# nv-tlabs/DiffusionTexturePainting

Hardware: AMD Instinct MI355X
Metric: 512x512 inpaint stamps/sec @20 DDIM steps (higher is better)
Workload: dtype f16

## Files before the change

### diffusiontexturepainting_amd/csrc/common.h

```cpp
#pragma once
#include <hip/hip_runtime.h>
#include <stdint.h>

#include "../../include/dtp.h"

typedef _Float16 f16;
typedef f16 f16x2 __attribute__((ext_vector_type(2)));
typedef f16 f16x4 __attribute__((ext_vector_type(4)));
typedef f16 f16x8 __attribute__((ext_vector_type(8)));
typedef float f32x4 __attribute__((ext_vector_type(4)));
typedef float f32x16 __attribute__((ext_vector_type(16)));

static __device__ __forceinline__ uint32_t lds_addr(const void* p) {
  return (uint32_t)(uintptr_t)(const __attribute__((address_space(3))) void*)p;
}
static __device__ __forceinline__ f16x8 lds_read16(uint32_t addr) {
  f16x8 v;
  asm volatile("ds_read_b128 %0, %1" : "=v"(v) : "v"(addr));
  return v;
}
template <int N, int NF>
static __device__ __forceinline__ void wait_lds_frags(f16x8 (&f)[NF]) {
  static_assert(NF == 2 || NF == 3 || NF == 4 || NF == 5 || NF == 6 || NF == 7 || NF == 8, "fragment count");
  if constexpr (NF == 2) asm volatile("s_waitcnt lgkmcnt(%2)" : "+v"(f[0]), "+v"(f[1]) : "n"(N));
  else if constexpr (NF == 3) asm volatile("s_waitcnt lgkmcnt(%3)" : "+v"(f[0]), "+v"(f[1]), "+v"(f[2]) : "n"(N));
  else if constexpr (NF == 4) asm volatile("s_waitcnt lgkmcnt(%4)" : "+v"(f[0]), "+v"(f[1]), "+v"(f[2]), "+v"(f[3]) : "n"(N));
  else if constexpr (NF == 5)
    asm volatile("s_waitcnt lgkmcnt(%5)" : "+v"(f[0]), "+v"(f[1]), "+v"(f[2]), "+v"(f[3]), "+v"(f[4]) : "n"(N));
  else if constexpr (NF == 6)
    asm volatile("s_waitcnt lgkmcnt(%6)" : "+v"(f[0]), "+v"(f[1]), "+v"(f[2]), "+v"(f[3]), "+v"(f[4]), "+v"(f[5]) : "n"(N));
  else if constexpr (NF == 7)
    asm volatile("s_waitcnt lgkmcnt(%7)"
                 : "+v"(f[0]), "+v"(f[1]), "+v"(f[2]), "+v"(f[3]), "+v"(f[4]), "+v"(f[5]), "+v"(f[6])
                 : "n"(N));
  else
    asm volatile("s_waitcnt lgkmcnt(%8)"
                 : "+v"(f[0]), "+v"(f[1]), "+v"(f[2]), "+v"(f[3]), "+v"(f[4]), "+v"(f[5]), "+v"(f[6]), "+v"(f[7])
                 : "n"(N));
}



#ifndef DTP_IEEE_DIV
static __device__ __forceinline__ float fast_rcp(float x) { return __builtin_amdgcn_rcpf(x); }
#else
static __device__ __forceinline__ float fast_rcp(float x) { return 1.0f / x; }
#endif
static __device__ __forceinline__ float silu_f(float x) { return x * fast_rcp(1.0f + __expf(-x)); }
static __device__ __forceinline__ float quick_gelu_f(float x) { return x * fast_rcp(1.0f + __expf(-1.702f * x)); }

#ifndef DTP_GELU_POLY
static __device__ __forceinline__ float gelu_erf(float x) {
  const float z = fabsf(x) * 0.70710678118654752f;
  const float t = fast_rcp(fmaf(0.3275911f, z, 1.0f));
  float pl = fmaf(1.061405429f, t, -1.453152027f);
  pl = fmaf(pl, t, 1.421413741f);
  pl = fmaf(pl, t, -0.284496736f);
  pl = fmaf(pl, t, 0.254829592f);
  const float e = 1.0f - pl * t * __expf(-z * z);
  return 0.5f * x * (1.0f + copysignf(e, x));
}
#else
static __device__ __forceinline__ float gelu_erf(float x) {
  const float z = fminf(fabsf(x) * 0.70710678118654752f, 3.0f);
  const float u = z * z;
  float p = fmaf(4.074155537e-08f, u, -1.944803169e-06f);
  p = fmaf(p, u, 4.106023957e-05f);
  p = fmaf(p, u, -5.110346811e-04f);
  p = fmaf(p, u, 4.235417930e-03f);
  p = fmaf(p, u, -2.510283806e-02f);
  p = fmaf(p, u, 1.110793054e-01f);
  p = fmaf(p, u, -3.753148582e-01f);
  p = fmaf(p, u, 1.128268424e+00f);
  const float h = 0.5f * x;
  return fmaf(fabsf(h), p * z, h);
}
#endif

typedef float f32x2 __attribute__((ext_vector_type(2)));
template <class T>
static __device__ __forceinline__ void sum_pairs_strided_t(const float* __restrict__ p, size_t stride, int n, T& s1, T& s2) {
  s1 = 0; s2 = 0;
  int q = 0;
  for (; q + 8 <= n; q += 8) {
    f32x2 t[8];
#pragma unroll
    for (int e = 0; e < 8; ++e) t[e] = *(const f32x2*)(p + (size_t)(q + e) * stride);
#pragma unroll
    for (int e = 0; e < 8; ++e) { s1 += (T)t[e][0]; s2 += (T)t[e][1]; }
  }
  if (q < n) {
    f32x2 t[8];
#pragma unroll
    for (int e = 0; e < 8; ++e) t[e] = *(const f32x2*)(p + (size_t)(q + (q + e < n ? e : 0)) * stride);
#pragma unroll
    for (int e = 0; e < 8; ++e)
      if (q + e < n) { s1 += (T)t[e][0]; s2 += (T)t[e][1]; }
  }
}
static __device__ __forceinline__ void sum_pairs_strided(const float* __restrict__ p, size_t stride, int n, float& s1, float& s2) {
  sum_pairs_strided_t(p, stride, n, s1, s2);
}
static __device__ __forceinline__ void sum_pairs_strided_d(const float* __restrict__ p, size_t stride, int n, double& s1, double& s2) {
  sum_pairs_strided_t(p, stride, n, s1, s2);
}
static __device__ __forceinline__ f32x4 col4(const float* __restrict__ v, int n, int N) {
  if (n + 4 <= N) return *(const f32x4*)(v + n);
  f32x4 r = {0.f, 0.f, 0.f, 0.f};
#pragma unroll
  for (int e = 0; e < 4; ++e)
    if (n + e < N) r[e] = v[n + e];
  return r;
}
static __device__ __forceinline__ double shfl_xor_d(double v, int o) {
  int lo = __double2loint(v), hi = __double2hiint(v);
  lo = __shfl_xor(lo, o); hi = __shfl_xor(hi, o);
  return __hiloint2double(hi, lo);
}
template <int CTRL>
static __device__ __forceinline__ float dpp_get_f(float v) {
  return __builtin_bit_cast(float, __builtin_amdgcn_update_dpp(0, __builtin_bit_cast(int, v), CTRL, 0xf, 0xf, false));
}
static __device__ __forceinline__ void swap16_f(float x, float& a, float& b) {
  a = x; b = x;
  asm volatile("s_nop 1\n\tv_permlane16_swap_b32 %0, %1" : "+v"(a), "+v"(b));
}
static __device__ __forceinline__ void swap32_f(float x, float& a, float& b) {
  a = x; b = x;
  asm volatile("s_nop 1\n\tv_permlane32_swap_b32 %0, %1" : "+v"(a), "+v"(b));
}
template <int W>
static __device__ __forceinline__ float group_allsum(float v) {
  static_assert(W == 2 || W == 4 || W == 8 || W == 16 || W == 32 || W == 64, "group width");
  v += dpp_get_f<0xb1>(v);
  if constexpr (W >= 4) v += dpp_get_f<0x4e>(v);
  if constexpr (W >= 8) v += dpp_get_f<0x141>(v);
  if constexpr (W >= 16) v += dpp_get_f<0x140>(v);
  if constexpr (W >= 32) { float a, b; swap16_f(v, a, b); v = a + b; }
  if constexpr (W >= 64) { float a, b; swap32_f(v, a, b); v = a + b; }
  return v;
}
template <int W>
static __device__ __forceinline__ float group_allmax(float v) {
  static_assert(W == 2 || W == 4 || W == 8 || W == 16, "group width");
  v = fmaxf(v, dpp_get_f<0xb1>(v));
  if constexpr (W >= 4) v = fmaxf(v, dpp_get_f<0x4e>(v));
  if constexpr (W >= 8) v = fmaxf(v, dpp_get_f<0x141>(v));
  if constexpr (W >= 16) v = fmaxf(v, dpp_get_f<0x140>(v));
  return v;
}
static __device__ __forceinline__ float xhalf_sum(float v) { float a, b; swap32_f(v, a, b); return a + b; }
static __device__ __forceinline__ float xhalf_max(float v) { float a, b; swap32_f(v, a, b); return fmaxf(a, b); }

template <int CTRL>
static __device__ __forceinline__ double dpp_add8_d(double v) {
  const int lo = __builtin_amdgcn_update_dpp(0, __double2loint(v), CTRL, 0xf, 0xf, false);
  const int hi = __builtin_amdgcn_update_dpp(0, __double2hiint(v), CTRL, 0xf, 0xf, false);
  return v + __hiloint2double(hi, lo);
}
static __device__ __forceinline__ double sum8_d(double v) {
  v = dpp_add8_d<0xb1>(v);
  v = dpp_add8_d<0x4e>(v);
  v = dpp_add8_d<0x141>(v);
  return v;
}
static __device__ __forceinline__ void gn_mean_rstd(double s, double q, float inv_count, float eps, float& mean, float& rstd) {
  const float nf = rintf(1.0f / inv_count);
  const double n = (double)nf;
  double inv = (double)(1.0f / nf);
  inv = inv * (2.0 - n * inv);
  const double m = s * inv;
  const double var = q * inv - m * m;
  mean = (float)m;
  rstd = rsqrtf(fmaxf((float)var, 0.f) + eps);
}

#define DTP_WAVE 64

#define HIP_CHECK(x)                                                                        \
  do {                                                                                      \
    hipError_t e_ = (x);                                                                    \
    if (e_ != hipSuccess) {                                                                 \
      dtp_set_error("%s:%d %s -> %s", __FILE__, __LINE__, #x, hipGetErrorString(e_));       \
      return DTP_ERR_HIP;                                                                   \
    }                                                                                       \
  } while (0)


void dtp_set_error(const char* fmt, ...);

enum {
  GF_BIAS = 1,
  GF_BIAS_M = 2,
  GF_RESID = 4,
  GF_GEGLU = 8,
  GF_CONV3 = 16,
  GF_UPS2 = 32,
  GF_GELU = 64,
  GF_QUICKGELU = 128,
  GF_OUT_F32 = 256,
  GF_SILU = 512,
  GF_LNFOLD = 1024,
  GF_ROWSTATS = 2048,
  GF_SOFTMAX16 = 4096,
  GF_MFAST = 1 << 20,
  GF_NOREDUCE = 1 << 21,
  GF_XCDSPLIT = 1 << 23,
  GF_GNSTATS = 1 << 24,
  GF_RAGGED = 1 << 25,
  GF_GNAPPLY = 1 << 22,
};

struct GemmParams {
  const f16* A;
  const f16* W;
  const f16* Wcb;
  const f16* Wfr;
  void* C;
  float* part;
  const float* bias;
  const f16* R;
  const f16* zero;
  const float* lns;
  float ln_eps;
  const float* st_in;
  int st_parts;
  float* st_out;
  int M, N, K;
  int lda, ldw, ldc, ldr;
  int nkb;
  int splits;
  int kb_per_split;
  int col_ranges;
  int Hi, Wi, Ho, Wo, Cin, stride, pad;
  const f16* A2;
  int lda2, Cin2;
  int flags;
  int batch;
  long long a_bs, w_bs, c_bs, r_bs;
  int bias_bs, lns_bs, st_rows;
  int sm_valid;
  const float *gn_part, *gn_gamma, *gn_beta;
  int gn_nchunk, gn_cpg, gn_silu;
  float gn_eps;
  const unsigned char* W8;
  int ldw8;
  float a_scale, w_scale;
  const float* a_scale_host;
  int amax_slot1;
  const unsigned char* A8;
  int lda8;
  const unsigned char* A2_8;
  int lda2_8;
  unsigned char* C8;
  int ldc8;
  float c_scale;
  float a2_scale;
};

struct Quant8Job {
  const f16* x; int ld, K;
  unsigned char* y; int ldy;
  float scale;
  int ln;
};
struct Quant8Params {
  int M, njobs;
  Quant8Job job[2];
  const float* st_in; int st_parts, st_rows;
  float eps;
};
bool dtp_quant8_supported(const Quant8Params& q);
int dtp_launch_quant8(const Quant8Params& q, hipStream_t s);
bool dtp_gemm_f8f8_supported(const GemmParams& p);
int dtp_gemm_f8f8_pick(const GemmParams& p, int num_cu);
int dtp_launch_gemm_f8f8(const GemmParams& p, int tile, hipStream_t s);
void dtp_gemm_f8f8_init();

static inline bool dtp_xcd_split_ok(int tiles, int splits) {
  if (splits < 2 || (splits & (splits - 1)) || splits > 32) return false;
  return splits >= 8 || (tiles % (8 / splits)) == 0;
}
static __device__ __forceinline__ void dtp_xcd_split(int id, int tiles, int splits, int& tile, int& z) {
  const int xcd = id & 7, idx = id >> 3;
  if (splits >= 8) { const int r = splits >> 3; z = xcd + 8 * (idx % r); tile = idx / r; }
  else { const int g = 8 / splits; z = xcd % splits; tile = idx * g + xcd / splits; }
}

int dtp_launch_gemm(const GemmParams& p, int tile, hipStream_t s);
void dtp_gemm_init();
int dtp_launch_tile(const GemmParams& p, int tile, hipStream_t s);
int dtp_launch_splitk_reduce(const GemmParams& p, hipStream_t s);
size_t dtp_gemm_workspace_bytes(const GemmParams& p);
void dtp_gemm_pick(GemmParams& p, int* tile, int num_cu);

struct GnParams {
  const f16* x; int ldx; f16* y; int ldy; const float *gamma, *beta; int B, HW, C, groups; float eps; int silu;
};
struct GnReduceSrc {
  const float* part; int splits; long long slab; int ldp; const float* bias; const f16* R; int ldr;
};
int dtp_launch_groupnorm(const GnParams& p, float* stats_ws, hipStream_t s);
size_t dtp_groupnorm_ws_bytes(int B, int HW, int C, int groups);
int dtp_groupnorm_stat_chunks(int HW);
int dtp_launch_groupnorm_apply(const GnParams& p, const float* partial, int nchunk, hipStream_t s);
int dtp_launch_groupnorm_stats(const GnParams& p, float* ws, const GnReduceSrc* rd, hipStream_t s);
bool dtp_reduce_groupnorm_supported(int HW, int C, int groups);
int dtp_launch_reduce_groupnorm(const GnParams& p, const GnReduceSrc& rd, int Cx, float* stats_ws, hipStream_t s);
bool dtp_groupnorm_reduce_accepts(int C, int groups, int ldx, int ldp, int ldr);
int dtp_launch_gn_fold_weights(const GnParams& p, const float* partial, int nchunk, const f16* W, int ldw, const float* bias, int Nout, f16* Wout,
                               long long w_bs, float* bias_out, int bias_bs, hipStream_t s);
int dtp_launch_layernorm(const f16* x, int ldx, f16* y, int ldy, const float* gamma, const float* beta, int rows, int C,
                         float eps, hipStream_t s);
int dtp_launch_softmax_rows(const f16* x, int ldx, f16* y, int ldy, int rows, int cols, float scale, hipStream_t s);

struct AttnParams {
  const f16 *Q, *K, *V;
  f16* O;
  int ldq, ldk, ldv, ldo;
  int B, H, Sq, Skv, D;
  long long qbs, kbs, vbs, obs;
  float scale;
  int prio;
  int skew;
};
int dtp_launch_attention(const AttnParams& p, hipStream_t s);
bool dtp_attention_uses_dma(const AttnParams& p);
bool dtp_attention_dma_supported(const AttnParams& p);
int dtp_launch_attention_dma(const AttnParams& p, hipStream_t s, int nw_force = 0);
int dtp_launch_attention_fp8(const AttnParams& p, float q_scale, float v_scale, hipStream_t s);

struct XattnParams {
  const f16* X; int ldx;
  const f16* W1; long long w1_bs;
  const float *b1, *lns1;
  const float* st_in; int st_parts, st_rows; float ln_eps;
  const f16* W2; long long w2_bs;
  const float* b2;
  const f16* R; int ldr;
  f16* Y; int ldy;
  float* st_out;
  int S, C, N, sm_valid;
  const f16* zero;
  int ct;
};
int dtp_xattn_tiles_per_wg(int S, int C, int N);
bool dtp_xattn_supported(const XattnParams& p);
int dtp_launch_xattn(const XattnParams& p, hipStream_t s);
void dtp_xattn_init();

struct XchainParams {
  const f16* A; int lda;
  const f16* Wo; int ldwo;
  const float* bo;
  const f16* Y; int ldy;
  const f16* W1; long long w1_bs;
  const float *b1, *lns1;
  const f16* W2; long long w2_bs;
  const float* b2;
  f16* Y3; int ldy3;
  float* st_out;
  int S, C, N, sm_valid;
  float ln_eps;
  int dup;
};
bool dtp_xchain_supported(const XchainParams& p);
int dtp_launch_xchain(const XchainParams& p, hipStream_t s);
void dtp_xchain_init();

struct FfchainParams {
  const f16* X; int ldx;
  const f16* W1; int ldw1;
  const float *lns1, *b1;
  const f16* Wm; int ldwm;
  const float* bm;
  const f16* R; int ldr;
  f16* Out; int ldo;
  int M, C;
  float ln_eps;
};
bool dtp_ffchain_supported(const FfchainParams& p);
int dtp_launch_ffchain(const FfchainParams& p, hipStream_t s);
void dtp_ffchain_init();

int dtp_launch_concat_channels(const f16* a, int lda, int Ca, const f16* b, int ldb, int Cb, f16* y, int ldy, long long rows,
                               hipStream_t s);
#define DTP_COPY_SEGS 8
struct CopySegs {
  int n;
  const char* src[DTP_COPY_SEGS];
  char* dst[DTP_COPY_SEGS];
  long long rows[DTP_COPY_SEGS], row_bytes[DTP_COPY_SEGS], src_stride[DTP_COPY_SEGS], dst_stride[DTP_COPY_SEGS];
  long long chunks[DTP_COPY_SEGS], total;
};
int dtp_launch_copy_rows(CopySegs segs, hipStream_t s);
int dtp_launch_f32_to_f16(const float* x, f16* y, long long n, hipStream_t s);
int dtp_launch_nchw_f32_to_nhwc_f16(const float* x, f16* y, int B, int C, int HW, int Cpad, hipStream_t s);
int dtp_launch_nhwc_f16_to_nchw_f32(const f16* x, int ldx, float* y, int B, int C, int HW, hipStream_t s);
int dtp_launch_pack_conv_weight(const float* w, f16* out, int Cout, int Cin, int Cin_pad, int taps, int ldw, hipStream_t s);
int dtp_launch_pack_linear_weight(const float* w, f16* out, int N, int K, int ldw, const int* row_map, hipStream_t s);
int dtp_launch_rowdot(const float* w, const float* v, float* out, int N, int K, hipStream_t s);
int dtp_launch_scale_cols(float* w, const float* g, int N, int K, hipStream_t s);
int dtp_launch_rowsum_f16(const f16* w, int ld, int K, float* out, int rows, hipStream_t s);
int dtp_launch_matmul_f32(const float* A, const float* B, float* C, int M, int N, int K, hipStream_t s);
int dtp_launch_expand_kv(const f16* kv, f16* kexp, f16* vexp, int N, int T, int C, int H, float scale, hipStream_t s);
int dtp_launch_transpose_f16(const f16* src, int lds_, f16* dst, int ldd, int rows, int cols, hipStream_t s);
int dtp_launch_rowdot_f16(const f16* a, int ld, const float* v, float* out, int rows, int K, hipStream_t s);
bool dtp_gemm_fp8_supported(const GemmParams& p);
int dtp_launch_gemm_fp8(const GemmParams& p, int tile, hipStream_t s);
void dtp_gemm_fp8_init();
int dtp_quantize_weights_fp8(const f16* w, int ldw, int K, int rows, unsigned char* out, int ldw8, float* scale_out, hipStream_t s);
bool dtp_gemm_wide_supported(const GemmParams& p, int variant);
int dtp_launch_gemm_wide(const GemmParams& p, int variant, hipStream_t s);
void dtp_gemm_wide_init();
constexpr int DTP_TILE_LNLIN = 50;
constexpr int DTP_TILE_WS0 = 51;
constexpr int DTP_WS_VARIANTS = 4;
constexpr int DTP_TILE_GEMMWS = 55;
constexpr int DTP_TILE_IDS = 56;

enum { PK_GEMM0 = 0, PK_ATTN = 12, PK_GN = 13, PK_LN = 14, PK_ELEM = 15, PK_SOFTMAX = 16, PK_HALO0 = 17, PK_BIG0 = 21, PK_WIDE0 = 25, PK_FP8 = 27, PK_KH2 = 28, PK_LW = 36, PK_XATTN = 44, PK_HALO3 = 45, PK_LNLIN = 47, PK_WS0 = 48, PK_GEMMWS = 52, PK_F8F8 = 53, PK_QUANT8 = 54, PK_COUNT = 55 };

enum DtpFamily : unsigned char { TF_NONE, TF_GEMM, TF_HALO, TF_WIDE, TF_FP8, TF_LNLIN, TF_CONVWS, TF_GEMMWS };
enum DtpSplit : unsigned char {
  SPLIT_K,
  SPLIT_HALO,
  SPLIT_BLOCKS,
  SPLIT_COLS,
  SPLIT_NONE,
};
struct DtpTile {
  DtpFamily fam;
  int var;
  int bm, bn, ns;
  int kh, lw;
  DtpSplit split;
  int pk;
};
inline DtpTile dtp_tile(int id) {
  static constexpr int sm[4] = {128, 128, 64, 64}, sn[4] = {128, 64, 64, 128};
  const int s = id & 3;
  if (id >= 0 && id < 12) return {TF_GEMM, 0, sm[s], sn[s], 2 + id / 4, 1, 0, SPLIT_K, PK_GEMM0 + id};
  if (id >= 12 && id < 16) return {TF_HALO, id - 12, 0, 0, 0, 0, 0, SPLIT_HALO, PK_HALO0 + id - 12};
  if (id >= 16 && id < 20) return {TF_GEMM, 0, id < 18 ? 256 : 128, id < 18 ? 128 : 256, 2 + (id & 1), 1, 0, SPLIT_K, PK_BIG0 + id - 16};
  if (id == 20 || id == 21) return {TF_WIDE, id - 20, 256, id == 20 ? 256 : 320, 2, 0, 0, SPLIT_NONE, PK_WIDE0 + id - 20};
  if (id >= 24 && id < 28) return {TF_FP8, id - 24, sm[s], sn[s], 2, 0, 0, SPLIT_NONE, PK_FP8};
  if (id == 28) return {TF_FP8, 4, 256, 256, 2, 0, 0, SPLIT_NONE, PK_FP8};
  if (id >= 32 && id < 40) return {TF_GEMM, 0, sm[s], sn[s], 2 + (id - 32) / 4, 2, 0, SPLIT_K, PK_KH2 + id - 32};
  if (id >= 40 && id < 48) return {TF_GEMM, 0, sm[s], sn[s], 3, 1, id < 44 ? 4 : 8, SPLIT_K, PK_LW + id - 40};
  if (id == 48 || id == 49) return {TF_HALO, id - 44, 0, 0, 0, 0, 0, SPLIT_HALO, PK_HALO3 + id - 48};
  if (id == DTP_TILE_LNLIN) return {TF_LNLIN, 0, 0, 0, 0, 0, 0, SPLIT_COLS, PK_LNLIN};
  if (id >= DTP_TILE_WS0 && id < DTP_TILE_WS0 + DTP_WS_VARIANTS) return {TF_CONVWS, id - DTP_TILE_WS0, 0, 0, 0, 0, 0, SPLIT_BLOCKS, PK_WS0 + id - DTP_TILE_WS0};
  if (id == DTP_TILE_GEMMWS) return {TF_GEMMWS, 0, 64, 64, 0, 0, 0, SPLIT_BLOCKS, PK_GEMMWS};
  return {};
}
inline bool dtp_tile_apply(GemmParams& p, int tile, int sp) {
  const DtpTile t = dtp_tile(tile);
  if (sp < 1) sp = 1;
  if (t.fam == TF_HALO) p.W = p.Wcb;
  if (t.split == SPLIT_NONE || t.split == SPLIT_COLS) {
    p.kb_per_split = p.nkb; p.splits = 1;
    if (t.split == SPLIT_COLS) p.col_ranges = sp;
    return t.split == SPLIT_COLS || sp == 1;
  }
  p.kb_per_split = (p.nkb + sp - 1) / sp;
  if (t.split == SPLIT_BLOCKS) { p.splits = sp; return true; }
  if (t.split == SPLIT_HALO && sp > 1) p.kb_per_split = (((p.nkb + 8) / 9 + sp - 1) / sp) * 9;
// ... 32 lines not shown
```

### diffusiontexturepainting_amd/csrc/conv_ws.hip

```cpp
#include <stdlib.h>
#include <type_traits>

#include "common.h"

namespace {

typedef __attribute__((address_space(3))) void* lds_ptr_t;
typedef unsigned int u32x4 __attribute__((ext_vector_type(4)));

template <int OFF>
__device__ __forceinline__ f16x8 lds_read16_off(uint32_t addr) {
  f16x8 v;
  asm volatile("ds_read_b128 %0, %1 offset:%2" : "=v"(v) : "v"(addr), "n"(OFF));
  return v;
}
template <int N>
__device__ __forceinline__ void wait_vmcnt() { asm volatile("s_waitcnt vmcnt(%0)" ::"n"(N) : "memory"); }

template <int TH, int TW, int NI, int NT, bool CO = false>
struct WsGeom {
  static constexpr int PW = TW + 3, PH = TH + 2;
  static constexpr int HP1 = PH * PW, HP = NI * HP1;
  static constexpr int HL = (HP + 31) / 32;
  static constexpr int PBYTES = HL * 32 * 128;
  static constexpr int TM = NI * TH * TW / 32;
  static constexpr int RPT = 32 / TW, TPI = TH / RPT;
  static constexpr int CBLK = 1152;
  static constexpr int CMB = 4 * (CO ? 1 : NT) * TM * 4 * CBLK;
  static constexpr int MAINB = (3 * PBYTES > CMB ? 3 * PBYTES : CMB);
  static constexpr int STATB = (NI == 1 && NT == 2) ? (4 * NT * 32 * 2 + NT * 32 * 2) * 8 : 0;
  static constexpr int LDS = MAINB + STATB;
  static constexpr int LT = (HL - 1) / (NT * TM);
  static constexpr int WAITB = (17 - LT) * NT;
  static_assert(TW == 8 || TW == 16, "pixel tile width");
  static_assert(TH % RPT == 0 && (NI * TH * TW) % 32 == 0, "whole MFMA tiles");
  static_assert(HP * 128 < 65536, "fragment offsets are 16-bit immediates");
  static_assert(LT < 8 && WAITB < 64, "patch pieces fit in the taps before the barrier; vmcnt is a 6-bit counter");
  static_assert(LDS <= (CO ? 80 : 160) * 1024, "LDS");
};

__global__ void pack_conv_ws_kernel(const float* __restrict__ w, f16* __restrict__ out, int Cout, int Cin, long long total) {
  for (long long i = (long long)blockIdx.x * 256 + threadIdx.x; i < total; i += (long long)gridDim.x * 256) {
    const int e = (int)(i & 7), l = (int)((i >> 3) & 63);
    long long f = i >> 9;
    const int tap = (int)(f % 9); f /= 9;
    const int wq = (int)(f & 3); f >>= 2;
    const int ncb = Cin >> 6;
    const int cb = (int)(f % ncb), nt = (int)(f / ncb);
    const int n = nt * 32 + (l & 31), ch = cb * 64 + 16 * wq + 8 * (l >> 5) + e;
    out[i] = n < Cout ? (f16)w[((size_t)n * Cin + ch) * 9 + tap] : (f16)0.f;
  }
}

__global__ void pack_conv_ws_tail_kernel(const float* __restrict__ w, f16* __restrict__ out, int Cout, int Cin2, long long total) {
  for (long long i = (long long)blockIdx.x * 256 + threadIdx.x; i < total; i += (long long)gridDim.x * 256) {
    const int e = (int)(i & 7), l = (int)((i >> 3) & 63);
    long long g = i >> 9;
    const int wq = (int)(g & 3); g >>= 2;
    const int ntb = Cin2 >> 6;
    const int tb = (int)(g % ntb), nt = (int)(g / ntb);
    const int n = nt * 32 + (l & 31), ch = tb * 64 + 16 * wq + 8 * (l >> 5) + e;
    out[i] = n < Cout ? (f16)w[(size_t)n * Cin2 + ch] : (f16)0.f;
  }
}

template <class G, int KY, int J>
__device__ __forceinline__ void rd_frags(f16x8 (&dst)[G::TM], uint32_t ct) {
  if constexpr (J < G::TM) {
    dst[J] = lds_read16_off<((J / G::TPI) * G::HP1 + (G::RPT * (J % G::TPI) + KY) * G::PW) * 128>(ct);
    rd_frags<G, KY, J + 1>(dst, ct);
  }
}

template <int TH, int TW, int NI, int NT, bool NTW, bool CO = false, bool RAG = false>
__global__ __launch_bounds__(256, CO ? 2 : 1) void convws_kernel(const GemmParams p) {
  using G = WsGeom<TH, TW, NI, NT, CO>;
  constexpr int TM = G::TM, HL = G::HL, PW = G::PW, PH = G::PH, HP1 = G::HP1, PB = G::PBYTES, NTM = NT * TM;
  extern __shared__ __attribute__((aligned(16))) char smem[];

  const int tid = threadIdx.x, lane = tid & 63;
  const int wave = __builtin_amdgcn_readfirstlane(tid >> 6);
  const int frow = lane & 31, fhalf = lane >> 5;

  const int H = p.Ho, W = p.Wo;
  const int tiles_x = RAG ? (W + TW - 1) / TW : W / TW, tiles_y = RAG ? (H + TH - 1) / TH : H / TH;
  const int hw = H * W;
  const bool pow2 = ((hw & (hw - 1)) | (tiles_x & (tiles_x - 1)) | (tiles_y & (tiles_y - 1))) == 0;
  const int images = pow2 ? (p.M >> __builtin_ctz(hw)) : p.M / hw;
  const int npg = (images / NI) * tiles_y * tiles_x;
  const int nts = (p.N + 31) >> 5, nrs = (nts + NT - 1) / NT, S = p.splits;
  const int units = nrs * S;
  const int xcd = blockIdx.x & 7, idx = blockIdx.x >> 3;
  int pg, u;
  if ((units & 7) == 0) { const int q = idx / npg; pg = idx - q * npg; u = q * 8 + xcd; }
  else { const int pgq = (npg + 7) >> 3; const int q = idx / pgq; pg = (idx - q * pgq) * 8 + xcd; u = q; }
  if (u >= units || pg >= npg) return;
  const int ncb = p.Cin >> 6;
  int z = 0, nr = u, mb0 = 0, mb1 = ncb;
  if (S > 1) {
    nr = u / S; z = u - nr * S;
    mb0 = z * ncb / S; mb1 = (z + 1) * ncb / S;
  }
  int tx, ty, img0;
  if (pow2) {
    const int sx = __builtin_ctz(tiles_x), sy = __builtin_ctz(tiles_y);
    tx = pg & (tiles_x - 1); ty = (pg >> sx) & (tiles_y - 1); img0 = (pg >> (sx + sy)) * NI;
  } else {
    tx = pg % tiles_x; ty = (pg / tiles_x) % tiles_y; img0 = (pg / (tiles_x * tiles_y)) * NI;
  }
  const int y0 = ty * TH, x0 = tx * TW;

  const auto rsW = __builtin_amdgcn_make_buffer_rsrc((void*)p.Wfr, 0, (int)0x80000000u, 0x00020000);
  constexpr int OOB = (int)0x80000000u;
  int wvoff[NT], wbase[NT];
#pragma unroll
  for (int i = 0; i < NT; ++i) {
    const int nt = nr * NT + i;
    wvoff[i] = nt < nts ? lane * 16 : OOB;
    wbase[i] = (nt < nts ? nt : 0) * ncb * 4 + wave;
  }
  auto wload = [&](int i, int cb, int tap) -> f16x8 {
    const u32x4 v = __builtin_amdgcn_raw_buffer_load_b128(rsW, wvoff[i], ((wbase[i] + cb * 4) * 9 + tap) * 1024, NTW ? 2 : 0);
    return __builtin_bit_cast(f16x8, v);
  };
  f16x8 wf[NT][9];
  if (mb0 < mb1) {
#pragma unroll
    for (int t = 0; t < 9; ++t)
#pragma unroll
      for (int i = 0; i < NT; ++i) wf[i][t] = wload(i, mb0, t);
  }
  __builtin_amdgcn_sched_barrier(0);

  const auto rsA = __builtin_amdgcn_make_buffer_rsrc((void*)p.A, 0, (int)0x80000000u, 0x00020000);
  int voffA[HL];
  {
    const int ups = (p.flags & GF_UPS2) ? 1 : 0;
    const int s0 = wave * 8 + (lane >> 3);
    int il = 0, hy = s0 / PW, hx = s0 - hy * PW;
    constexpr int DY = 32 / PW, DX = 32 - DY * PW;
#pragma unroll
    for (int i = 0; i < HL; ++i) {
      const int iy = y0 + hy - 1, ix = x0 + hx - 1;
      const bool ok = il < NI && hx < TW + 2 && (unsigned)iy < (unsigned)H && (unsigned)ix < (unsigned)W;
      voffA[i] = ok ? ((((img0 + il) * p.Hi + (iy >> ups)) * p.Wi + (ix >> ups)) * p.lda + (((lane & 7) ^ (hx & 7)) << 3)) * 2 : -1;
      hx += DX; hy += DY;
      if (hx >= PW) { hx -= PW; ++hy; }
      if (hy >= PH) { hy -= PH; ++il; }
    }
  }
  auto a_piece_at = [&](uint32_t bo, int cb, int i) {
    const int vo = voffA[i];
    __builtin_amdgcn_raw_ptr_buffer_load_lds(rsA, (lds_ptr_t)(smem + bo + (i * 4 + wave) * 1024), 16, vo, cb * 128, 0, 0);
  };
  if (mb0 < mb1) {
#pragma unroll
    for (int i = 0; i < HL; ++i) a_piece_at(0u, mb0, i);
    if (mb0 + 1 < mb1) {
#pragma unroll
      for (int i = 0; i < HL; ++i) a_piece_at((uint32_t)PB, mb0 + 1, i);
    }
  }

  const int pxl = frow % TW, pyl = frow / TW;
  uint32_t colterm[3];
#pragma unroll
  for (int kx = 0; kx < 3; ++kx)
    colterm[kx] = lds_addr(smem) + (pyl * PW + pxl + kx) * 128 + ((((2 * wave + fhalf) ^ ((pxl + kx) & 7))) << 4);

  f32x16 acc[NT][TM];
#pragma unroll
  for (int i = 0; i < NT; ++i)
#pragma unroll
    for (int j = 0; j < TM; ++j)
#pragma unroll
      for (int r = 0; r < 16; ++r) acc[i][j][r] = 0.f;

  constexpr int NBF = CO ? 2 : 3;
  f16x8 bf[NBF][TM];
  auto rd = [&](auto tapc, uint32_t bo, f16x8 (&dst)[TM]) {
    constexpr int TAP = decltype(tapc)::value, KY = TAP / 3, KX = TAP % 3;
#ifndef DTP_WS_NO_LDSREAD
    rd_frags<G, KY, 0>(dst, colterm[KX] + bo);
#else
#pragma unroll
    for (int j = 0; j < TM; ++j) asm volatile("" : "+v"(dst[j]));
#endif
  };
  if (mb0 < mb1 && !(p.sm_valid & 1)) {
    wait_vmcnt<0>();
    __builtin_amdgcn_s_barrier();
    rd(std::integral_constant<int, 0>{}, 0u, bf[0]);
    auto do_cb = [&](auto morec, auto more2c, int cb, uint32_t bo, uint32_t bo1, uint32_t bo2) {
      constexpr bool MORE = decltype(morec)::value, MORE2 = decltype(more2c)::value;
      auto tap = [&](auto tapc) {
        constexpr int TAP = decltype(tapc)::value, CUR = TAP % NBF, NXT = (TAP + 1) % NBF;
        __builtin_amdgcn_sched_barrier(0);
#ifdef DTP_WS_NO_LDSREAD
#define DTP_WS_WAIT(n, f) asm volatile("" ::: "memory")
#else
#define DTP_WS_WAIT(n, f) wait_lds_frags<n, TM>(f)
#endif
        if constexpr (TAP < 8) {
          rd(std::integral_constant<int, TAP + 1>{}, bo, bf[NXT]);
          __builtin_amdgcn_sched_barrier(0);
          DTP_WS_WAIT(TM, bf[CUR]);
        } else {
          DTP_WS_WAIT(0, bf[CUR]);
          if constexpr (MORE) {
            wait_vmcnt<G::WAITB>();
            __builtin_amdgcn_s_barrier();
            if constexpr (!CO) {
              rd(std::integral_constant<int, 0>{}, bo1, bf[NXT]);
              __builtin_amdgcn_sched_barrier(0);
            }
          }
        }
#pragma unroll
        for (int j = 0; j < TM; ++j)
#pragma unroll
          for (int i = 0; i < NT; ++i) {
#ifndef DTP_WS_NO_MFMA
            acc[i][j] = __builtin_amdgcn_mfma_f32_32x32x16_f16(wf[i][TAP], bf[CUR][j], acc[i][j], 0, 0, 0);
#else
            asm volatile("" : "+v"(acc[i][j]) : "v"(wf[i][TAP]), "v"(bf[CUR][j]));
#endif
            if constexpr (MORE2) {
              if (TAP * NTM + j * NT + i < HL) {
                __builtin_amdgcn_sched_barrier(0);
#ifndef DTP_WS_NO_DMA
                a_piece_at(bo2, cb + 2, TAP * NTM + j * NT + i);
#endif
                __builtin_amdgcn_sched_barrier(0);
              }
            }
          }
        if constexpr (MORE) {
          __builtin_amdgcn_sched_barrier(0);
#ifndef DTP_WS_NO_WLOAD
#pragma unroll
          for (int i = 0; i < NT; ++i) wf[i][TAP] = wload(i, cb + 1, TAP);
#endif
          __builtin_amdgcn_sched_barrier(0);
          if constexpr (CO && TAP == 8) rd(std::integral_constant<int, 0>{}, bo1, bf[0]);
        }
      };
#undef DTP_WS_WAIT
      tap(std::integral_constant<int, 0>{}); tap(std::integral_constant<int, 1>{}); tap(std::integral_constant<int, 2>{});
      tap(std::integral_constant<int, 3>{}); tap(std::integral_constant<int, 4>{}); tap(std::integral_constant<int, 5>{});
      tap(std::integral_constant<int, 6>{}); tap(std::integral_constant<int, 7>{}); tap(std::integral_constant<int, 8>{});
    };
    typedef std::true_type Y;
    typedef std::false_type N_;
    uint32_t bo = 0, bo1 = PB, bo2 = 2 * PB;
    int cb = mb0;
    for (; cb + 2 < mb1; ++cb) {
      do_cb(Y{}, Y{}, cb, bo, bo1, bo2);
      const uint32_t t = bo; bo = bo1; bo1 = bo2; bo2 = t;
    }
    if (cb + 1 < mb1) {
      do_cb(Y{}, N_{}, cb, bo, bo1, bo2);
      ++cb;
      bo = bo1;
    }
    do_cb(N_{}, N_{}, cb, bo, bo1, bo2);
  }

  if (p.A2 && !(p.sm_valid & 1)) {
    const int ntb = p.Cin2 >> 6;
    const int tk0 = (int)((long long)z * ntb / S), tk1 = (int)((long long)(z + 1) * ntb / S);
    if (tk0 < tk1) {
      const auto rsT = __builtin_amdgcn_make_buffer_rsrc((void*)p.A2, 0, (int)0x80000000u, 0x00020000);
      int voffT[TM];
#pragma unroll
      for (int j = 0; j < TM; ++j) {
        const int il = j / G::TPI, py = G::RPT * (j % G::TPI) + pyl;
        voffT[j] = ((((img0 + il) * H + y0 + py) * W + x0 + pxl) * p.lda2 + 8 * fhalf) * 2;
        if (RAG && (y0 + py >= H || x0 + pxl >= W)) voffT[j] = OOB;
      }
      int tbase[NT];
#pragma unroll
      for (int i = 0; i < NT; ++i) tbase[i] = nts * ncb * 36 + (nr * NT + i < nts ? nr * NT + i : 0) * ntb * 4;
      constexpr int D = CO ? 2 : (TM % 4 == 0) ? 4 : 3;
      static_assert(TM % D == 0, "tile ring");
      f16x8 ring[4 * D];
      constexpr int WTB = CO ? 1 : 2;
      f16x8 wt[WTB][NT][4];
      auto frag_load = [&](int tb, int j, int slot) {
        const int vo = tb < tk1 ? voffT[j] : OOB;
#pragma unroll
        for (int ks = 0; ks < 4; ++ks) {
          const u32x4 v = __builtin_amdgcn_raw_buffer_load_b128(rsT, vo, tb * 128 + ks * 32, 0);
          ring[slot * 4 + ks] = __builtin_bit_cast(f16x8, v);
        }
      };
      auto wt_load = [&](int tb, int par) {
#pragma unroll
        for (int i = 0; i < NT; ++i) {
          const int vo = tb < tk1 ? wvoff[i] : OOB;
#pragma unroll
          for (int ks = 0; ks < 4; ++ks) {
            const u32x4 v = __builtin_amdgcn_raw_buffer_load_b128(rsW, vo, (tbase[i] + tb * 4 + ks) * 1024, NTW ? 2 : 0);
            wt[par % WTB][i][ks] = __builtin_bit_cast(f16x8, v);
          }
        }
      };
      const int nround = (tk1 - tk0 + 3) >> 2;
      int tb = tk0 + wave;
      wt_load(tb, 0);
#pragma unroll
      for (int j = 0; j < D; ++j) frag_load(tb, j, j);
      auto block = [&](auto parc, int tbc, bool more) {
        constexpr int PAR = decltype(parc)::value % WTB;
        if (WTB == 2 && more) wt_load(tbc + 4, PAR ^ 1);
#pragma unroll
        for (int j = 0; j < TM; ++j) {
#pragma unroll
          for (int ks = 0; ks < 4; ++ks)
#pragma unroll
            for (int i = 0; i < NT; ++i)
              acc[i][j] = __builtin_amdgcn_mfma_f32_32x32x16_f16(wt[PAR][i][ks], ring[(j % D) * 4 + ks], acc[i][j], 0, 0, 0);
          if (j + D < TM) frag_load(tbc, j + D, j % D);
          else if (more) frag_load(tbc + 4, j + D - TM, j % D);
        }
        if (WTB == 1 && more) wt_load(tbc + 4, 0);
      };
      for (int r = 0; r < nround; r += 2) {
        block(std::integral_constant<int, 0>{}, tb, r + 1 < nround);
        if (r + 1 < nround) block(std::integral_constant<int, 1>{}, tb + 4, r + 2 < nround);
        tb += 8;
      }
    }
  }

  if (p.sm_valid & 2) return;
  __builtin_amdgcn_s_barrier();
  constexpr int CB = G::CBLK;
  constexpr int RT = CO ? 1 : NT;
  const int epx = tid >> 3, c4 = tid & 7;
  const int epxl = epx % TW, epyl = epx / TW;
  const char* const src0 = smem + (c4 >> 1) * CB + ((epx * 2 + (c4 & 1)) ^ ((epx >> 2) & 1)) * 16;
  constexpr bool CAN_STATS = G::STATB > 0;
  const bool stats = CAN_STATS && (p.flags & GF_GNSTATS) && p.splits == 1;
  double* const sred = (double*)(smem + G::MAINB);
#pragma unroll
  for (int i0 = 0; i0 < NT; i0 += RT) {
    if (i0 > 0) __syncthreads();
    {
      char* const mine = smem + wave * RT * TM * 4 * CB + ((frow * 2 + fhalf) ^ ((frow >> 2) & 1)) * 16;
#pragma unroll
      for (int i = 0; i < RT; ++i)
#pragma unroll
        for (int j = 0; j < TM; ++j)
#pragma unroll
          for (int q = 0; q < 4; ++q) {
            const f32x4 v = {acc[i0 + i][j][4 * q], acc[i0 + i][j][4 * q + 1], acc[i0 + i][j][4 * q + 2], acc[i0 + i][j][4 * q + 3]};
            *(f32x4*)(mine + ((i * TM + j) * 4 + q) * CB) = v;
          }
    }
    __syncthreads();
#pragma unroll
    for (int i = 0; i < RT; ++i) {
      const int n = (nr * NT + i0 + i) * 32 + 4 * c4;
      const bool ncol = n + 4 <= p.N;
      f32x4 bv = {0.f, 0.f, 0.f, 0.f};
      if (p.splits == 1 && (p.flags & GF_BIAS) && ncol) bv = *(const f32x4*)(p.bias + n);
      float ssum[4] = {0.f, 0.f, 0.f, 0.f}, qsum[4] = {0.f, 0.f, 0.f, 0.f};
#pragma unroll
      for (int j = 0; j < TM; ++j) {
        const char* src = src0 + (i * TM + j) * 4 * CB;
        const f32x4 v0 = *(const f32x4*)src, v1 = *(const f32x4*)(src + RT * TM * 4 * CB), v2 = *(const f32x4*)(src + 2 * RT * TM * 4 * CB),
                    v3 = *(const f32x4*)(src + 3 * RT * TM * 4 * CB);
        f32x4 v;
#pragma unroll
        for (int e = 0; e < 4; ++e) v[e] = ((v0[e] + v1[e]) + v2[e]) + v3[e];
        const int il = j / G::TPI, py = G::RPT * (j % G::TPI) + epyl;
        if (RAG && (y0 + py >= H || x0 + epxl >= W)) continue;
        const size_t m = ((size_t)(img0 + il) * H + y0 + py) * W + x0 + epxl;
        if (!ncol) continue;
        if (p.splits > 1) {
          *(f32x4*)(p.part + ((size_t)z * p.M + m) * p.N + n) = v;
        } else {
#pragma unroll
          for (int e = 0; e < 4; ++e) v[e] += bv[e];
          if (p.flags & GF_RESID) {
            const f16x4 r = *(const f16x4*)(p.R + m * p.ldr + n);
#pragma unroll
            for (int e = 0; e < 4; ++e) v[e] += (float)r[e];
          }
          const f16x4 o = {(f16)v[0], (f16)v[1], (f16)v[2], (f16)v[3]};
          *(f16x4*)((f16*)p.C + m * p.ldc + n) = o;
          if constexpr (CAN_STATS) {
#pragma unroll
            for (int e = 0; e < 4; ++e) { const float f = (float)o[e]; ssum[e] += f; qsum[e] += f * f; }
          }
        }
      }
      if constexpr (CAN_STATS) {
        if (stats) {
          double sd[4], qd[4];
#pragma unroll
          for (int e = 0; e < 4; ++e) {
            sd[e] = (double)ssum[e]; qd[e] = (double)qsum[e];
#pragma unroll
            for (int o = 8; o < 64; o <<= 1) { sd[e] += shfl_xor_d(sd[e], o); qd[e] += shfl_xor_d(qd[e], o); }
          }
          if (lane < 8) {
            double* d = sred + ((wave * NT + i0 + i) * 32 + 4 * c4) * 2;
#pragma unroll
            for (int e = 0; e < 4; ++e) { d[2 * e] = sd[e]; d[2 * e + 1] = qd[e]; }
          }
        }
      }
    }
  }
  if constexpr (CAN_STATS) {
    if (stats) {
      __syncthreads();
      double* const tot = sred + 4 * NT * 32 * 2;
      if (tid < NT * 32 * 2) tot[tid] = ((sred[tid] + sred[NT * 64 + tid]) + sred[2 * NT * 64 + tid]) + sred[3 * NT * 64 + tid];
      __syncthreads();
      const int cpg = p.gn_cpg, groups = p.N / cpg;
      const int c_lo = nr * NT * 32, c_hi = min(p.N, c_lo + NT * 32);
      const int g_lo = c_lo / cpg, g_hi = (c_hi - 1) / cpg;
      const int g = g_lo + tid;
      if (g <= g_hi) {
        const int a = max(g * cpg, c_lo), b = min((g + 1) * cpg, c_hi);
        double sg = 0.0, qg = 0.0;
        for (int c = a; c < b; ++c) { sg += tot[(c - c_lo) * 2]; qg += tot[(c - c_lo) * 2 + 1]; }
        const int ntile = tiles_x * tiles_y, pt = ty * tiles_x + tx;
        float* const base = p.st_out + ((size_t)img0 * 2 * ntile + 2 * pt) * groups * 2;
        float* const mine = base + (size_t)(nr & 1) * groups * 2 + g * 2;
        mine[0] = (float)sg; mine[1] = (float)qg;
        if (g * cpg >= c_lo && (g + 1) * cpg <= c_hi) {
          float* const other = base + (size_t)((nr & 1) ^ 1) * groups * 2 + g * 2;
          other[0] = 0.f; other[1] = 0.f;
        }
      }
    }
  }
}

template <int TH, int TW, int NI, int NT, bool CO = false>
int launch_ws(const GemmParams& p, hipStream_t s) {
  using G = WsGeom<TH, TW, NI, NT, CO>;
  const bool rag = (p.Ho % TH) || (p.Wo % TW);
  const int npg = (p.M / (p.Ho * p.Wo) / NI) * ((p.Ho + TH - 1) / TH) * ((p.Wo + TW - 1) / TW);
  const int nrs = (((p.N + 31) >> 5) + NT - 1) / NT;
  const int units = nrs * p.splits;
  const int blocks = (units & 7) == 0 ? units * npg : ((npg + 7) >> 3) * 8 * units;
  static const int dbg = [] { const char* e = getenv("DTP_WS_DEBUG"); return e ? atoi(e) : 0; }();
  GemmParams q = p;
  q.sm_valid = dbg & 3;
  const bool nt = (dbg & 4) ? false : (dbg & 8) ? true : npg == 1;
  if constexpr (NI == 1 && NT == 2) {
    if (rag) {
      if (nt) hipLaunchKernelGGL((convws_kernel<TH, TW, NI, NT, true, CO, true>), dim3(blocks), dim3(256), G::LDS, s, q);
      else hipLaunchKernelGGL((convws_kernel<TH, TW, NI, NT, false, CO, true>), dim3(blocks), dim3(256), G::LDS, s, q);
      return hipGetLastError() == hipSuccess ? DTP_OK : DTP_ERR_HIP;
    }
  }
  if (nt) hipLaunchKernelGGL((convws_kernel<TH, TW, NI, NT, true, CO>), dim3(blocks), dim3(256), G::LDS, s, q);
  else hipLaunchKernelGGL((convws_kernel<TH, TW, NI, NT, false, CO>), dim3(blocks), dim3(256), G::LDS, s, q);
  return hipGetLastError() == hipSuccess ? DTP_OK : DTP_ERR_HIP;
}

template <int TH, int TW, int NI, int NT, bool CO = false>
void set_ws_attr() {
  (void)hipFuncSetAttribute((const void*)convws_kernel<TH, TW, NI, NT, true, CO>, hipFuncAttributeMaxDynamicSharedMemorySize, WsGeom<TH, TW, NI, NT, CO>::LDS);
  (void)hipFuncSetAttribute((const void*)convws_kernel<TH, TW, NI, NT, false, CO>, hipFuncAttributeMaxDynamicSharedMemorySize, WsGeom<TH, TW, NI, NT, CO>::LDS);
  if constexpr (NI == 1 && NT == 2) {
    (void)hipFuncSetAttribute((const void*)convws_kernel<TH, TW, NI, NT, true, CO, true>, hipFuncAttributeMaxDynamicSharedMemorySize, WsGeom<TH, TW, NI, NT, CO>::LDS);
    (void)hipFuncSetAttribute((const void*)convws_kernel<TH, TW, NI, NT, false, CO, true>, hipFuncAttributeMaxDynamicSharedMemorySize, WsGeom<TH, TW, NI, NT, CO>::LDS);
  }
}

}

void dtp_conv_ws_init() {
  set_ws_attr<8, 8, 3, 1>();
  set_ws_attr<16, 16, 1, 1>();
  set_ws_attr<8, 16, 1, 2>();
  set_ws_attr<8, 16, 1, 2, true>();
}

int dtp_conv_ws_gn_chunks(int Ho, int Wo) { return 2 * ((Ho + 7) / 8) * ((Wo + 15) / 16); }

size_t dtp_conv_ws_packed_elems(int Cout, int Cin, int Cin2) { return (size_t)((Cout + 31) / 32) * ((size_t)(Cin / 64) * 36 + (size_t)(Cin2 / 64) * 4) * 512; }

int dtp_launch_pack_conv_ws(const float* w, const float* w1, f16* out, int Cout, int Cin, int Cin2, hipStream_t s) {
  if ((Cin & 63) || (Cin2 & 63) || (Cin2 > 0) != (w1 != nullptr)) { dtp_set_error("pack_conv_ws: Cin %d / Cin2 %d must be multiples of 64", Cin, Cin2); return DTP_ERR_ARG; }
  const long long total = (long long)dtp_conv_ws_packed_elems(Cout, Cin, 0);
  const int blocks = (int)((total + 255) / 256 > 65535 ? 65535 : (total + 255) / 256);
  hipLaunchKernelGGL(pack_conv_ws_kernel, dim3(blocks), dim3(256), 0, s, w, out, Cout, Cin, total);
  if (Cin2 > 0) {
    const long long t2 = (long long)dtp_conv_ws_packed_elems(Cout, 0, Cin2);
    const int b2 = (int)((t2 + 255) / 256 > 65535 ? 65535 : (t2 + 255) / 256);
    hipLaunchKernelGGL(pack_conv_ws_tail_kernel, dim3(b2), dim3(256), 0, s, w1, out + total, Cout, Cin2, t2);
  }
  return hipGetLastError() == hipSuccess ? DTP_OK : DTP_ERR_HIP;
}

bool dtp_conv_ws_supported(const GemmParams& p, int variant, int nsplit) {
  if (!p.Wfr || !(p.flags & GF_CONV3) || p.batch > 1) return false;
  if (p.A2 && ((p.Cin2 & 63) || (p.lda2 & 7) || (size_t)p.M * p.lda2 * 2 >= ((size_t)1 << 31))) return false;
  if (p.flags & (GF_GEGLU | GF_OUT_F32 | GF_LNFOLD | GF_ROWSTATS | GF_BIAS_M | GF_GELU | GF_QUICKGELU | GF_SILU | GF_GNAPPLY | GF_SOFTMAX16)) return false;
  if (p.stride != 1 || p.pad != 1 || (p.Cin & 63) || (p.N & 3) || (p.lda & 7) || (p.ldc & 3)) return false;
  const bool rag = (p.flags & GF_RAGGED) != 0;
  if (p.flags & GF_UPS2) {
    if ((p.Ho != 2 * p.Hi && !(rag && p.Ho == 2 * p.Hi - 1)) || (p.Wo != 2 * p.Wi && !(rag && p.Wo == 2 * p.Wi - 1))) return false;
  }
  else if (p.Ho != p.Hi || p.Wo != p.Wi) return false;
  if ((p.flags & GF_RESID) && (p.ldr & 3)) return false;
  if (p.Ho < 1 || p.Wo < 1 || p.M % (p.Ho * p.Wo)) return false;
  const int images = p.M / (p.Ho * p.Wo);
  if (variant == 0) { if (p.Ho != 8 || p.Wo != 8 || images % 3) return false; }
  else if (variant == 1) { if (p.Ho != 16 || p.Wo != 16) return false; }
  else if (variant == 2 || variant == 3) { if (((p.Ho & 7) || (p.Wo & 15)) && !rag) return false; }
  else return false;
  if (p.flags & GF_GNSTATS) {
    if (variant < 2 || nsplit != 1 || !p.st_out || p.gn_cpg < 4 || p.gn_cpg > 64 || (p.N % p.gn_cpg) || p.N / p.gn_cpg > 32) return false;
  }
  if (nsplit < 1 || nsplit > p.Cin / 64) return false;
  if ((size_t)images * p.Hi * p.Wi * p.lda * 2 >= ((size_t)1 << 31) || dtp_conv_ws_packed_elems(p.N, p.Cin, p.A2 ? p.Cin2 : 0) * 2 >= ((size_t)1 << 31)) return false;
  return true;
}

int dtp_launch_conv_ws(const GemmParams& pin, int variant, hipStream_t s) {
  if (!dtp_conv_ws_supported(pin, variant, pin.splits)) {
    dtp_set_error("conv_ws: unsupported problem (M %d N %d Cin %d %dx%d flags %#x, variant %d, %d slices)", pin.M, pin.N, pin.Cin, pin.Hi, pin.Wi, pin.flags, variant, pin.splits);
    return DTP_ERR_ARG;
  }
  const int rc = variant == 0 ? launch_ws<8, 8, 3, 1>(pin, s) : variant == 1 ? launch_ws<16, 16, 1, 1>(pin, s) : variant == 2 ? launch_ws<8, 16, 1, 2>(pin, s) : launch_ws<8, 16, 1, 2, true>(pin, s);
  if (rc != DTP_OK) { dtp_set_error("conv_ws launch failed: %s", hipGetErrorString(hipGetLastError())); return rc; }
  if (pin.splits > 1 && !(pin.flags & GF_NOREDUCE)) return dtp_launch_splitk_reduce(pin, s);
  return DTP_OK;
}
```

Before: 10.47.

## Prefetch epilogue bias, residual and shortcut operands during the final conv taps

Bias and residual loads for the epilogue are now issued as buffer loads inside the last channel block's nine-tap loop, so their latency overlaps the remaining MFMA work. The shortcut (A2) GEMM's first weight and fragment loads are also started during those taps. Under a compile-time flag, the GroupNorm stats cross-lane double reduction swaps shuffles for DPP and swizzle operations. This adds register pressure from the held residual and bias quads and shortcut buffers, which may reduce occupancy or cause spills.

```diff
diff --git a/diffusiontexturepainting_amd/csrc/common.h b/diffusiontexturepainting_amd/csrc/common.h
--- a/diffusiontexturepainting_amd/csrc/common.h
+++ b/diffusiontexturepainting_amd/csrc/common.h
@@ -163,6 +163,18 @@
   v = dpp_add8_d<0x4e>(v);
   v = dpp_add8_d<0x141>(v);
   return v;
+}
+static __device__ __forceinline__ double xor16_add_d(double v) {
+  float al, bl, ah, bh;
+  swap16_f(__int_as_float(__double2loint(v)), al, bl);
+  swap16_f(__int_as_float(__double2hiint(v)), ah, bh);
+  return __hiloint2double(__float_as_int(ah), __float_as_int(al)) + __hiloint2double(__float_as_int(bh), __float_as_int(bl));
+}
+static __device__ __forceinline__ double xor32_add_d(double v) {
+  float al, bl, ah, bh;
+  swap32_f(__int_as_float(__double2loint(v)), al, bl);
+  swap32_f(__int_as_float(__double2hiint(v)), ah, bh);
+  return __hiloint2double(__float_as_int(ah), __float_as_int(al)) + __hiloint2double(__float_as_int(bh), __float_as_int(bl));
 }
 static __device__ __forceinline__ void gn_mean_rstd(double s, double q, float inv_count, float eps, float& mean, float& rstd) {
   const float nf = rintf(1.0f / inv_count);
diff --git a/diffusiontexturepainting_amd/csrc/conv_ws.hip b/diffusiontexturepainting_amd/csrc/conv_ws.hip
--- a/diffusiontexturepainting_amd/csrc/conv_ws.hip
+++ b/diffusiontexturepainting_amd/csrc/conv_ws.hip
@@ -14,6 +14,10 @@
   asm volatile("ds_read_b128 %0, %1 offset:%2" : "=v"(v) : "v"(addr), "n"(OFF));
   return v;
 }
+#ifndef DTP_WS_TAIL
+#define DTP_WS_TAIL 15
+#endif
+
 template <int N>
 __device__ __forceinline__ void wait_vmcnt() { asm volatile("s_waitcnt vmcnt(%0)" ::"n"(N) : "memory"); }
 
@@ -178,6 +182,90 @@
 
   constexpr int NBF = CO ? 2 : 3;
   f16x8 bf[NBF][TM];
+
+  const int epx = tid >> 3, c4 = tid & 7;
+  const int epxl = epx % TW, epyl = epx / TW;
+  const bool ep_full = p.splits == 1;
+  f32x4 bvq[NT];
+  f16x4 rq[NT][TM];
+  const auto rsB = __builtin_amdgcn_make_buffer_rsrc((void*)p.bias, 0, (int)0x80000000u, 0x00020000);
+  const auto rsR = __builtin_amdgcn_make_buffer_rsrc((void*)p.R, 0, (int)0x80000000u, 0x00020000);
+  auto bias_req = [&](int i) {
+    const int n = (nr * NT + i) * 32 + 4 * c4;
+    const bool on = ep_full & ((p.flags & GF_BIAS) != 0) & (n + 4 <= p.N);
+    bvq[i] = __builtin_bit_cast(f32x4, __builtin_amdgcn_raw_buffer_load_b128(rsB, on ? n * 4 : OOB, 0, 0));
+  };
+  auto resid_req = [&](int i, int j, bool now) {
+    const int n = (nr * NT + i) * 32 + 4 * c4;
+    const int il = j / G::TPI, py = G::RPT * (j % G::TPI) + epyl;
+    const bool on = now & ep_full & ((p.flags & GF_RESID) != 0) & (n + 4 <= p.N) & !(RAG & ((y0 + py >= H) | (x0 + epxl >= W)));
+    const int m = ((img0 + il) * H + y0 + py) * W + x0 + epxl;
+    rq[i][j] = __builtin_bit_cast(f16x4, __builtin_amdgcn_raw_buffer_load_b64(rsR, ((m * p.ldr + n) * 2) | (on ? 0 : OOB), 0, 0));
+  };
+  const bool sc_on = p.A2 && !(p.sm_valid & 1);
+  const int ntb = sc_on ? p.Cin2 >> 6 : 0;
+  const int tk0 = (int)((long long)z * ntb / S), tk1 = (int)((long long)(z + 1) * ntb / S);
+  const auto rsT = __builtin_amdgcn_make_buffer_rsrc((void*)p.A2, 0, (int)0x80000000u, 0x00020000);
+  constexpr int D = CO ? 2 : (TM % 4 == 0) ? 4 : 3;
+  static_assert(TM % D == 0, "tile ring");
+  constexpr int WTB = CO ? 1 : 2;
+  constexpr int FSTEP = 1;
+  constexpr int SCF = (DTP_WS_TAIL & 4) && NT == 2 && !CO ? D : -1;
+  static_assert(4 + SCF * FSTEP <= 8, "the shortcut's first tiles are requested inside the nine taps");
+  f16x8 ring[4 * D];
+  f16x8 wt[WTB][NT][4];
+  int voffT[TM], tbase[NT];
+  auto sc_setup = [&]() {
+#pragma unroll
+    for (int j = 0; j < TM; ++j) {
+      const int il = j / G::TPI, py = G::RPT * (j % G::TPI) + pyl;
+      voffT[j] = ((((img0 + il) * H + y0 + py) * W + x0 + pxl) * p.lda2 + 8 * fhalf) * 2;
+      if (RAG && (y0 + py >= H || x0 + pxl >= W)) voffT[j] = OOB;
+    }
+#pragma unroll
+    for (int i = 0; i < NT; ++i) tbase[i] = nts * ncb * 36 + (nr * NT + i < nts ? nr * NT + i : 0) * ntb * 4;
+  };
+  auto frag_load = [&](int tb, int j, int slot) {
+    const int vo = tb < tk1 ? voffT[j] : OOB;
+#pragma unroll
+    for (int ks = 0; ks < 4; ++ks) {
+      const u32x4 v = __builtin_amdgcn_raw_buffer_load_b128(rsT, vo, tb * 128 + ks * 32, 0);
+      ring[slot * 4 + ks] = __builtin_bit_cast(f16x8, v);
+    }
+  };
+  auto wt_load = [&](int tb, auto parc) {
+    constexpr int PAR = decltype(parc)::value % WTB;
+#pragma unroll
+    for (int i = 0; i < NT; ++i) {
+      const int vo = tb < tk1 ? wvoff[i] : OOB;
+#pragma unroll
+      for (int ks = 0; ks < 4; ++ks) {
+        const u32x4 v = __builtin_amdgcn_raw_buffer_load_b128(rsW, vo, (tbase[i] + tb * 4 + ks) * 1024, NTW ? 2 : 0);
+        wt[PAR][i][ks] = __builtin_bit_cast(f16x8, v);
+      }
+    }
+  };
+  auto tail_req = [&](auto tapc) {
+    constexpr int TAP = decltype(tapc)::value;
+    if constexpr ((DTP_WS_TAIL & 1) && NT == 2 && TAP == 0) {
+#pragma unroll
+      for (int i = 0; i < NT; ++i) bias_req(i);
+    }
+    if constexpr ((DTP_WS_TAIL & 2) && NT == 2 && !CO && TAP >= 1) {
+#pragma unroll
+      for (int k = 0; k < 2 * NT; ++k) {
+        constexpr int Q0 = (TAP - 1) * 2 * NT;
+        if (Q0 + k < NTM) resid_req((Q0 + k) / TM, (Q0 + k) % TM, !p.A2);
+      }
+    }
+    if constexpr (SCF >= 0 && TAP >= 4) {
+      if (tk0 < tk1) {
+        if constexpr (TAP == 4) { sc_setup(); wt_load(tk0 + wave, std::integral_constant<int, 0>{}); }
+        if constexpr (TAP > 4 && (TAP - 4) % FSTEP == 0 && (TAP - 4) / FSTEP <= SCF) frag_load(tk0 + wave, (TAP - 4) / FSTEP - 1, (TAP - 4) / FSTEP - 1);
+      }
+    }
+  };
+  static_assert(TM <= 16, "the residual quads are requested inside the nine taps");
   auto rd = [&](auto tapc, uint32_t bo, f16x8 (&dst)[TM]) {
     constexpr int TAP = decltype(tapc)::value, KY = TAP / 3, KX = TAP % 3;
 #ifndef DTP_WS_NO_LDSREAD
@@ -243,6 +331,10 @@
 #endif
           __builtin_amdgcn_sched_barrier(0);
           if constexpr (CO && TAP == 8) rd(std::integral_constant<int, 0>{}, bo1, bf[0]);
+        } else {
+          __builtin_amdgcn_sched_barrier(0);
+          tail_req(tapc);
+          asm volatile("" ::: "memory");
         }
       };
 #undef DTP_WS_WAIT
@@ -264,55 +356,25 @@
       bo = bo1;
     }
     do_cb(N_{}, N_{}, cb, bo, bo1, bo2);
-  }
-
-  if (p.A2 && !(p.sm_valid & 1)) {
-    const int ntb = p.Cin2 >> 6;
-    const int tk0 = (int)((long long)z * ntb / S), tk1 = (int)((long long)(z + 1) * ntb / S);
+  } else {
+    tail_req(std::integral_constant<int, 0>{}); tail_req(std::integral_constant<int, 1>{}); tail_req(std::integral_constant<int, 2>{});
+    tail_req(std::integral_constant<int, 3>{}); tail_req(std::integral_constant<int, 4>{}); tail_req(std::integral_constant<int, 5>{});
+    tail_req(std::integral_constant<int, 6>{}); tail_req(std::integral_constant<int, 7>{}); tail_req(std::integral_constant<int, 8>{});
+  }
+
+  {
     if (tk0 < tk1) {
-      const auto rsT = __builtin_amdgcn_make_buffer_rsrc((void*)p.A2, 0, (int)0x80000000u, 0x00020000);
-      int voffT[TM];
-#pragma unroll
-      for (int j = 0; j < TM; ++j) {
-        const int il = j / G::TPI, py = G::RPT * (j % G::TPI) + pyl;
-        voffT[j] = ((((img0 + il) * H + y0 + py) * W + x0 + pxl) * p.lda2 + 8 * fhalf) * 2;
-        if (RAG && (y0 + py >= H || x0 + pxl >= W)) voffT[j] = OOB;
-      }
-      int tbase[NT];
-#pragma unroll
-      for (int i = 0; i < NT; ++i) tbase[i] = nts * ncb * 36 + (nr * NT + i < nts ? nr * NT + i : 0) * ntb * 4;
-      constexpr int D = CO ? 2 : (TM % 4 == 0) ? 4 : 3;
-      static_assert(TM % D == 0, "tile ring");
-      f16x8 ring[4 * D];
-      constexpr int WTB = CO ? 1 : 2;
-      f16x8 wt[WTB][NT][4];
-      auto frag_load = [&](int tb, int j, int slot) {
-        const int vo = tb < tk1 ? voffT[j] : OOB;
-#pragma unroll
-        for (int ks = 0; ks < 4; ++ks) {
-          const u32x4 v = __builtin_amdgcn_raw_buffer_load_b128(rsT, vo, tb * 128 + ks * 32, 0);
-          ring[slot * 4 + ks] = __builtin_bit_cast(f16x8, v);
-        }
-      };
-      auto wt_load = [&](int tb, int par) {
-#pragma unroll
-        for (int i = 0; i < NT; ++i) {
-          const int vo = tb < tk1 ? wvoff[i] : OOB;
-#pragma unroll
-          for (int ks = 0; ks < 4; ++ks) {
-            const u32x4 v = __builtin_amdgcn_raw_buffer_load_b128(rsW, vo, (tbase[i] + tb * 4 + ks) * 1024, NTW ? 2 : 0);
-            wt[par % WTB][i][ks] = __builtin_bit_cast(f16x8, v);
-          }
-        }
-      };
       const int nround = (tk1 - tk0 + 3) >> 2;
       int tb = tk0 + wave;
-      wt_load(tb, 0);
-#pragma unroll
-      for (int j = 0; j < D; ++j) frag_load(tb, j, j);
+      if constexpr (SCF < 0) {
+        sc_setup();
+        wt_load(tb, std::integral_constant<int, 0>{});
+      }
+#pragma unroll
+      for (int j = SCF < 0 ? 0 : SCF; j < D; ++j) frag_load(tb, j, j);
       auto block = [&](auto parc, int tbc, bool more) {
         constexpr int PAR = decltype(parc)::value % WTB;
-        if (WTB == 2 && more) wt_load(tbc + 4, PAR ^ 1);
+        if (WTB == 2 && more) wt_load(tbc + 4, std::integral_constant<int, PAR ^ 1>{});
 #pragma unroll
         for (int j = 0; j < TM; ++j) {
 #pragma unroll
@@ -323,7 +385,7 @@
           if (j + D < TM) frag_load(tbc, j + D, j % D);
           else if (more) frag_load(tbc + 4, j + D - TM, j % D);
         }
-        if (WTB == 1 && more) wt_load(tbc + 4, 0);
+        if (WTB == 1 && more) wt_load(tbc + 4, std::integral_constant<int, 0>{});
       };
       for (int r = 0; r < nround; r += 2) {
         block(std::integral_constant<int, 0>{}, tb, r + 1 < nround);
@@ -334,11 +396,18 @@
   }
 
   if (p.sm_valid & 2) return;
+  if constexpr ((DTP_WS_TAIL & 1) && NT == 1) bias_req(0);
+  if constexpr ((DTP_WS_TAIL & 2) != 0) {
+    if (CO || NT == 1 || p.A2) {
+#pragma unroll
+      for (int i = 0; i < NT; ++i)
+#pragma unroll
+        for (int j = 0; j < TM; ++j) resid_req(i, j, true);
+    }
+  }
   __builtin_amdgcn_s_barrier();
   constexpr int CB = G::CBLK;
   constexpr int RT = CO ? 1 : NT;
-  const int epx = tid >> 3, c4 = tid & 7;
-  const int epxl = epx % TW, epyl = epx / TW;
   const char* const src0 = smem + (c4 >> 1) * CB + ((epx * 2 + (c4 & 1)) ^ ((epx >> 2) & 1)) * 16;
   constexpr bool CAN_STATS = G::STATB > 0;
   const bool stats = CAN_STATS && (p.flags & GF_GNSTATS) && p.splits == 1;
@@ -363,8 +432,8 @@
     for (int i = 0; i < RT; ++i) {
       const int n = (nr * NT + i0 + i) * 32 + 4 * c4;
       const bool ncol = n + 4 <= p.N;
-      f32x4 bv = {0.f, 0.f, 0.f, 0.f};
-      if (p.splits == 1 && (p.flags & GF_BIAS) && ncol) bv = *(const f32x4*)(p.bias + n);
+      if constexpr (!(DTP_WS_TAIL & 1)) bias_req(i0 + i);
+      const f32x4 bv = bvq[i0 + i];
       float ssum[4] = {0.f, 0.f, 0.f, 0.f}, qsum[4] = {0.f, 0.f, 0.f, 0.f};
 #pragma unroll
       for (int j = 0; j < TM; ++j) {
@@ -384,7 +453,8 @@
 #pragma unroll
           for (int e = 0; e < 4; ++e) v[e] += bv[e];
           if (p.flags & GF_RESID) {
-            const f16x4 r = *(const f16x4*)(p.R + m * p.ldr + n);
+            if constexpr (!(DTP_WS_TAIL & 2)) resid_req(i0 + i, j, true);
+            const f16x4 r = rq[i0 + i][j];
 #pragma unroll
             for (int e = 0; e < 4; ++e) v[e] += (float)r[e];
           }
@@ -402,8 +472,14 @@
 #pragma unroll
           for (int e = 0; e < 4; ++e) {
             sd[e] = (double)ssum[e]; qd[e] = (double)qsum[e];
+#if DTP_WS_TAIL & 8
+            sd[e] = dpp_add8_d<0x128>(sd[e]); qd[e] = dpp_add8_d<0x128>(qd[e]);
+            sd[e] = xor16_add_d(sd[e]); qd[e] = xor16_add_d(qd[e]);
+            sd[e] = xor32_add_d(sd[e]); qd[e] = xor32_add_d(qd[e]);
+#else
 #pragma unroll
             for (int o = 8; o < 64; o <<= 1) { sd[e] += shfl_xor_d(sd[e], o); qd[e] += shfl_xor_d(qd[e], o); }
+#endif
           }
           if (lane < 8) {
             double* d = sred + ((wave * NT + i0 + i) * 32 + 4 * c4) * 2;
@@ -511,7 +587,7 @@
     if ((p.Ho != 2 * p.Hi && !(rag && p.Ho == 2 * p.Hi - 1)) || (p.Wo != 2 * p.Wi && !(rag && p.Wo == 2 * p.Wi - 1))) return false;
   }
   else if (p.Ho != p.Hi || p.Wo != p.Wi) return false;
-  if ((p.flags & GF_RESID) && (p.ldr & 3)) return false;
+  if ((p.flags & GF_RESID) && ((p.ldr & 3) || (size_t)p.M * p.ldr * 2 >= ((size_t)1 << 31))) return false;
   if (p.Ho < 1 || p.Wo < 1 || p.M % (p.Ho * p.Wo)) return false;
   const int images = p.M / (p.Ho * p.Wo);
   if (variant == 0) { if (p.Ho != 8 || p.Wo != 8 || images % 3) return false; }
```

Measured after the change: 10.53 (median of 6 runs). No clear change (+0.6%).
